# sujeetv/parquet-go

Measured on AMD Instinct MI355X. Metric: decoded GB/s (uncompressed output) per GPU & node at 1/2/4/8; % HBM roofline, higher is better.
Workload: dtype int32; 1 GPU; C2: optional INT32, 100000000 rows x 7 dictionary widths (b=1,2,4,8,12,16,20), ~10% nulls, RLE_DICTIONARY (uniform indices), V1, UNCOMPRESSED, 20000 rows/page; bytes_in=821696760, bytes_out=3220121800, streams=2, parallelism=single GPU

## Files before the change

parquet-go_amd/csrc/pqg_kernels.h:

```cpp
#pragma once
#include <hip/hip_runtime.h>

#include "pqgpu.h"
#include "pqg_common.h"

namespace pqg {

namespace crc { struct Rec; struct TileRec; }
namespace flt { struct Pred; struct Col; struct Sel; }

constexpr int kCrcWaves = 4;
constexpr int kCrcThreads = 64 * kCrcWaves;
constexpr int kBigWaves = 8;
constexpr int kBigDictThreads = 64 * kBigWaves;
constexpr int kExportWaves = 4;
constexpr int kExportThreads = 64 * kExportWaves;
constexpr int kExportGridY = 16;
constexpr int kWalkLanes = kWalkThreads;

__global__ void k_tile_jobs(const JobDev* jobs, int* tile_job);
__global__ void k_page_cands(JobDev* jobs, const int* tile_job, int* tile_count, int* tile_okc, int64_t* cand_pos,
                             int* cand_list, int* cand_total, int region);
__global__ void k_cand_parse(JobDev* jobs, const int* tile_job, const int* cand_list, const int* cand_total, int region,
                             int* tile_okc, const int64_t* cand_pos, Cand* cands);
__global__ void k_tile_scan(JobDev* jobs, const int* tile_count, const int* tile_okc, int* tile_off, int* tile_okoff);
__global__ void k_cand_link(JobDev* jobs, const int* tile_job, int64_t total_tiles, const int* tile_count,
                            const int* tile_off, const int* tile_okoff, const Cand* cands, int* succ, int* idx2slot,
                            int* ok2slot);
__global__ void k_page_chain(JobDev* jobs, PageDev* pages, const Cand* cands, const int* succ, const int* idx2slot,
                             const int* ok2slot, int* order);
__global__ void k_scan_pages(JobDev* jobs, PageDev* pages, int n_jobs, int prewalk, int stride);
__global__ void k_page_list(JobDev* jobs, PageDev* pages, int n_jobs, int* list, int list_cap, int* total,
                            int* queues);
__global__ void k_crc_plan(const JobDev* jobs, const PageDev* pages, const int* list, const int* total, int n_recs,
                           crc::Rec* recs, crc::TileRec* tiles, int tile_cap, int* tile_ctr);
__global__ void k_page_crc(const crc::Rec* recs, const crc::TileRec* tiles, const int* tile_ctr, int tile_cap,
                           int* queue, uint32_t* raws);
__global__ void k_crc_fin(PageDev* pages, const int* list, const int* total, int n_recs, crc::Rec* recs,
                          const uint32_t* raws);
__global__ void k_snap_plan(const JobDev* jobs, PageDev* pages, const int* list, const int* total, int* ctr,
                            SnapSub* subs, int sub_cap, int* seg_page, int seg_cap);
__global__ void k_snap_seg(const JobDev* jobs, const PageDev* pages, const int* seg_page, const int* seg_total,
                           int seg_cap, uint2* F);
__global__ void k_snap_link(const JobDev* jobs, PageDev* pages, const int* list, const int* total, SnapSub* subs,
                            const uint2* F);
__global__ void k_snap_decode(const JobDev* jobs, PageDev* pages, const SnapSub* subs, const int* sub_total,
                              int sub_cap, int* queue, uint8_t* scratch);
__global__ void k_snappy(JobDev* jobs, PageDev* pages, const int* list, const int* total, int* queue,
                         uint8_t* scratch);
__global__ void k_inflate(JobDev* jobs, PageDev* pages, const int* list, const int* total, int* queue,
                          uint8_t* scratch, int mode);
__global__ void k_inflate_s(JobDev* jobs, PageDev* pages, const int* list, const int* total, int* queue,
                            uint8_t* scratch);
__global__ void k_zstd(JobDev* jobs, PageDev* pages, const int* list, const int* total, int* queue, uint8_t* scratch,
                       uint8_t* wspace);
__global__ void k_lz4(JobDev* jobs, PageDev* pages, const int* list, const int* total, int* queue, uint8_t* scratch);
__global__ void k_lz4_batch(JobDev* jobs, PageDev* pages, const int* list, const int* total, int* queue,
                            uint8_t* scratch);
__global__ void k_page_levels(JobDev* jobs, PageDev* pages, const int* list, const int* total, int* queue,
                              uint8_t* scratch, HStream* streams, uint8_t* def_arena, uint8_t* rep_arena,
                              LongLev* longs, int long_cap, LevPiece* pieces, int piece_cap, int split);
__global__ void k_page_levels_w1(JobDev* jobs, PageDev* pages, const int* list, const int* total, int* queue,
                                 uint8_t* scratch, HStream* streams, uint8_t* def_arena, uint8_t* rep_arena,
                                 LongLev* longs, int long_cap, LevPiece* pieces, int piece_cap, int split);
__global__ void k_dict_resolve(JobDev* jobs, int n_jobs, PageDev* pages, uint8_t* scratch);
__global__ void k_level_long(PageDev* pages, const int* ctr, const LongLev* longs, int long_cap,
                             const LevPiece* pieces, int piece_cap, int* queue);
__global__ void k_hybrid_walk(const PageDev* pages, const int* list, const int* total, HStream* streams,
                              RunEnt* runs, BlockDesc* blks, LongWalk* longs, int long_cap);
__global__ void k_walk_long(const int* ctr, const LongWalk* longs, int long_cap, BlockDesc* blks);
__global__ void k_nn_scan_sums(JobDev* jobs, PageDev* pages, uint8_t* scratch, const HStream* streams, NnSums* sums,
                               NnJob* njobs, int* ctr, int64_t parts_cap);
__global__ void k_nn_scan(JobDev* jobs, PageDev* pages, uint8_t* scratch, const HStream* streams, const BlockDesc* blks,
                          int* ctr, PartRec* parts, int64_t parts_cap, const NnSums* sums, const NnJob* njobs);
template <int Mode>
__global__ void k_values(JobDev* jobs, PageDev* pages, const PartRec* parts, const int* total, int* queue,
                         uint8_t* value_arena, const HStream* streams, const RunEnt* runs, const BlockDesc* blks);
__global__ void k_finalize(JobDev* jobs, int n_jobs, const PageDev* pages);
__global__ void k_bss(JobDev* jobs, PageDev* pages, const PartRec* parts, const int* total, int* queue,
                      uint8_t* value_arena);
__global__ void k_dict_idx(JobDev* jobs, PageDev* pages, const PartRec* parts, const int* total, int* queue,
                           uint8_t* value_arena, const HStream* streams, const RunEnt* runs, const BlockDesc* blks);
__global__ void k_dict_export(JobDev* jobs, const PageDev* pages, int64_t* aoffs_arena, uint8_t* dchars_arena);
__global__ void k_dict_plan(JobDev* jobs, PageDev* pages, const PartRec* parts, const int* total,
                            uint8_t* value_arena, const HStream* streams, const RunEnt* runs, const BlockDesc* blks,
                            VRec* recs);
__global__ void k_dict4(PageDev* pages, const int* total, int* queue, const VRec* recs, int big);
__global__ void k_dict4_big(PageDev* pages, const int* total, int* queue, const VRec* recs);
__global__ void k_str_dict(JobDev* jobs, PageDev* pages, int64_t* doffs_arena);
__global__ void k_str_count(JobDev* jobs, PageDev* pages, PartRec* parts, const int* total, int* queue,
                            int64_t* offs_arena, const HStream* streams, const RunEnt* runs, const BlockDesc* blks);
__global__ void k_str_plain(JobDev* jobs, PageDev* pages, const int* list, const int* total, int* queue,
                            int64_t* offs_arena);
__global__ void k_char_scan(JobDev* jobs, PageDev* pages, PartRec* parts, int64_t* offs_arena);
__global__ void k_str_delta(JobDev* jobs, PageDev* pages, const int* list, const int* total, int* queue,
                            int64_t* offs_arena);
__global__ void k_str_dba(JobDev* jobs, PageDev* pages, const int* list, const int* total, int* queue,
                          uint8_t* value_arena, int64_t* offs_arena);
__global__ void k_str_copy(JobDev* jobs, PageDev* pages, const PartRec* parts, const int* total, int* queue,
                           uint8_t* value_arena, int64_t* offs_arena);

int assemble_launch(hipStream_t s, const pqg_assemble_args* a, int64_t* seg_scratch, int64_t* tot);
int list_count_launch(hipStream_t s, const pqg_list_args* a, int64_t* seg_scratch, int64_t* tot);
int list_write_launch(hipStream_t s, const pqg_list_args* a, int64_t* seg_scratch);
int nested_count_launch(hipStream_t s, const pqg_nested_args* a, int64_t* seg_scratch, int64_t* tot);
int nested_write_launch(hipStream_t s, const pqg_nested_args* a, int64_t* seg_scratch, const int64_t* tot);
int pack_levels_launch(hipStream_t s, const uint8_t* levels, int64_t n, int bw, uint8_t* packed);
int filter_launch(hipStream_t s, const flt::Pred& p, const flt::Col& c, const pqg_dictionary* dict, uint32_t* ebits,
                  uint8_t* bitmap, int64_t n, int mode, bool lds, int64_t* seg, int64_t* tot);
int select_launch(hipStream_t s, const flt::Sel& a, int64_t* seg, int64_t* tot);

#ifdef PQG_PROFILE
int prof_read_values(unsigned long long* out);
int prof_read_levels(unsigned long long* out);
int prof_read_strings(unsigned long long* out);
int prof_read_snappy(unsigned long long* out);
int prof_read_dict(unsigned long long* out);
int prof_read_inflate(unsigned long long* out);
int prof_read_bss(unsigned long long* out);
#endif

}
```

parquet-go_amd/csrc/pqg_levdec.h:

```cpp
#pragma once
#include "pqg_common.h"
#include "pqg_device.h"
#include "pqg_hybrid.h"

namespace pqg {

__device__ __forceinline__ int reg_stream(const JobDev& job, const PageDev& pg, HStream* streams, int32_t* slot,
                                          int pidx, int kind, gcu8 p, int64_t n, int w, int64_t count) {
  const int64_t rb = pg.run_off, bb = pg.blk_off;
  const int id = pidx * 3 + (kind > 2 ? 2 : kind);
  HStream& S = streams[id];
  S.p = (const uint8_t*)p;
  S.n = n;
  S.run_base = job.run_base + rb;
  S.blk_base = job.blk_base + bb;
  S.page = pidx;
  S.kind = kind;
  S.w = w;
  S.count = (int32_t)count;
  S.n_runs = 0;
  S.produced = 0;
  S.status = kOK;
  S.n_blocks = 0;
  *slot = id;
// ... 513 lines not shown
        const uint32_t ok = pay < n ? (n - pay + (uint32_t)w - 1) / (uint32_t)w : 0u;
        take = ok * 8;
        status = kEOF;
      }
    }
    if (status != kOK) return status;
    if (take > (uint32_t)kLongLev && longs && defer_long(bp, take, pay, produced)) {
      deferred = true;
      produced += take;
      pos = nx;
      return kOK;
    }
    uint32_t done = 0;
    while (done < take) {
      const uint32_t pre = (uint32_t)(((uintptr_t)out + produced) & 15);
      uint32_t piece = take - done;
      if (piece > (uint32_t)kLSpan - pre) piece = (uint32_t)kLSpan - pre;
      uint32_t info = pay;
      if (bp) {
        const uint64_t b0 = (uint64_t)pay * 8 + (uint64_t)done * (uint32_t)w;
        const uint32_t byte0 = (uint32_t)(b0 >> 3);
        const uint32_t nbytes = (uint32_t)(((uint64_t)piece * (uint32_t)w + 7) >> 3) + 8;
        if (!in_win(byte0, nbytes)) fill(byte0);
        info = 0x80000000u | (uint32_t)(((uint64_t)(byte0 - wbase) << 3) + (b0 & 7));
      }
      if (kW1 || w == 1) {
        bits_clear();
        if ((uint32_t)lane <= (pre + piece - 1) >> 5) bits_or(pre, piece, bp, bp ? (info & 0x7fffffffu) : pay, lane);
        bits_store(produced, piece);
        produced += piece;
        done += piece;
        continue;
      }
      if constexpr (!kW1) {
      PQG_L uint8_t* TM = lds_ptr(sh->tmap);
      *(PQG_L u32x4_t*)(TM + 16 * lane) = u32x4_t{0u, 0u, 0u, 0u};
      __builtin_amdgcn_wave_barrier();
      if (lane == 0) {
        lds_ptr(sh->tent)[0] = u32x2_t{pre, info};
        TM[pre] = 1;
      }
      __builtin_amdgcn_wave_barrier();
      expand(produced, piece);
      produced += piece;
      done += piece;
      }
    }
    pos = nx;
    return kOK;
  }
};

struct LongTables {
  LongLev* longs;
  LevPiece* pieces;
  int* ctr;
  int long_cap, piece_cap;
};

using LevelDecoder = LevelDecoderT<false>;

template <bool kW1 = false>
__device__ __forceinline__ int level_stream(gcu8 p, int64_t n, int w, uint32_t count, gu8 out, uint32_t maxl,
                                            LevShared& sh, uint32_t* nn, const LongTables& lt, int pidx,
                                            bool* deferred = nullptr) {
  LevelDecoderT<kW1> dec{p, (uint32_t)n, kW1 ? 1 : w, count, out, maxl, &sh, lt.longs, lt.pieces, lt.ctr, lt.long_cap,
                         lt.piece_cap, pidx};
  const int e = dec.run();
#ifdef PQG_PROFILE
  for (int k = 0; k < 8; k++) PQG_ACC(k, 0, dec.pacc[k]);
#endif
  *nn = (uint32_t)wave_sum((int64_t)dec.nn);
  if (deferred) *deferred = dec.deferred;
  return e;
}

struct PageStreams {
  gcu8 rep, def;
  int64_t rep_n, def_n;
  int e;
  gcu8 val;
  int64_t val_n;
  int vmode;
};
__device__ __forceinline__ PageStreams page_setup(const JobDev& job, const PageDev& pg, int pidx, PageDev* pages,
                                                  HStream* streams, const int* total, const uint8_t* scratch,
                                                  bool writer) {
  PageStreams r{nullptr, nullptr, -1, -1, kOK, nullptr, 0, -1};
  gcu8 block;
  int64_t blen;
  int32_t levels = 0;
  if (pg.page_type == 3) {
    levels = (int32_t)((uint32_t)pg.rep_len + (uint32_t)pg.def_len);
    blen = (int32_t)((uint32_t)pg.csize - (uint32_t)levels);
    if (pg.scratch_offset >= 0) blen = (int32_t)((uint32_t)pg.usize - (uint32_t)levels);
  } else {
    blen = pg.scratch_offset >= 0 ? pg.usize : pg.csize;
  }
  if (pg.scratch_offset >= 0) block = gconst(scratch) + job.scratch_base + pg.scratch_offset;
  else block = gconst(job.data) + pg.payload_offset + (levels > 0 ? levels : 0);
  int64_t vpos = 0;
  if (pg.page_type == 0) {
    if (job.max_rep > 0) {
      if (blen - vpos < 4) r.e = kEOF;
      else {
        const int64_t sz = rd_u32(block + vpos);
        const int64_t take = min(sz, blen - vpos - 4);
        r.rep = block + vpos + 4;
        r.rep_n = take;
        vpos += 4 + take;
      }
    }
    if (r.e == kOK && job.max_def > 0) {
      if (blen - vpos < 4) r.e = kEOF;
      else {
        const int64_t sz = rd_u32(block + vpos);
        const int64_t take = min(sz, blen - vpos - 4);
        r.def = block + vpos + 4;
        r.def_n = take;
        vpos += 4 + take;
      }
    }
  } else {
    gcu8 lv = gconst(job.data) + pg.payload_offset;
    if (levels > 0 && pg.rep_len > 0) { r.rep = lv; r.rep_n = pg.rep_len; }
    if (levels > 0 && pg.def_len > 0) { r.def = lv + pg.rep_len; r.def_n = levels - pg.rep_len; }
  }
  if (r.e != kOK) {
    if (writer) pages[pidx].read_status = r.e;
    return r;
  }
  if (job.keep_dict && pg.encoding != 8) {
    r.e = kNOT_DICT;
    if (writer) pages[pidx].read_status = r.e;
    return r;
  }
  const int64_t n = pg.num_values;
  const int64_t vn = blen - vpos;
  gcu8 val = block + vpos;
  r.val = val;
  r.val_n = vn;
  r.vmode = job.keep_dict                                              ? kModeIdx
            : pg.encoding == 9 && job.value_width > 0                  ? kModeBss
            : job.value_width == 0 || (pg.encoding == 7 && job.type == 7) ? 2
            : (pg.encoding == 8 && job.value_width == 4)                ? 1
            : pg.encoding == 5                                          ? 3
                                                                        : 0;
  if (writer) {
    PageDev& P = pages[pidx];
    P.block = (const uint8_t*)block;
    P.block_len = blen;
    P.val = (const uint8_t*)val;
    P.val_n = vn;
    P.rep = (const uint8_t*)r.rep;
    P.rep_n = r.rep_n;
    P.def = (const uint8_t*)r.def;
    P.def_n = r.def_n;
    if (pg.encoding == 8 && vn >= 1) {
      const int wv = val[0];
      P.dict_width = wv;
      if (wv >= 1 && wv <= 32 && n > 0) reg_stream(job, pg, streams, &P.hs_val, pidx, 2, val + 1, vn - 1, wv, n);
    } else if (pg.encoding == 3 && job.type == 0 && vn >= 4) {
      const int64_t sz = rd_u32(val);
      const int64_t take = min(sz, vn - 4);
      if (n > 0) reg_stream(job, pg, streams, &P.hs_val, pidx, 3, val + 4, take, 1, n);
    }
    const int vm = r.vmode;
    P.vmode = vm;
    int* present = const_cast<int*>(total) + kModePresentOff;
    if (present[vm] == 0) present[vm] = 1;
    if (vm == 2 && (pg.encoding == 6 || pg.encoding == 7) && present[kPresentDeltaStr] == 0) present[kPresentDeltaStr] = 1;
  }
  return r;
}

}
```

parquet-go_amd/csrc/pqg_levels.hip:

```cpp
#include <hip/hip_runtime.h>

#include "pqg_common.h"
#include "pqg_kernels.h"
#include "pqg_device.h"
#include "pqg_hybrid.h"
#include "pqg_levdec.h"
#include "pqg_lev1.h"
#include <type_traits>

namespace pqg {

#ifndef PQG_LEVELS_WPE
#define PQG_LEVELS_WPE 6
#endif

#ifdef PQG_PROFILE
int prof_read_levels(unsigned long long* out) {
  unsigned long long z[64] = {0};
  if (hipMemcpyFromSymbol(out, HIP_SYMBOL(pqg_prof), sizeof(z)) != hipSuccess) return -1;
  hipMemcpyToSymbol(HIP_SYMBOL(pqg_prof), z, sizeof(z));
  return 0;
}
#endif


#ifndef PQG_LANE_WIN
#define PQG_LANE_WIN 8
#endif
constexpr int kLaneWinG = PQG_LANE_WIN;
struct LaneWin {
  gcu8 p;
  uint32_t n;
  uint32_t base;
  PQG_L uint32_t* r;
  __device__ __forceinline__ void fill(uint32_t pos) {
    const uint32_t mis = (uint32_t)((uintptr_t)(p + pos) & 15);
    base = pos - mis;
    const uintptr_t a0 = (uintptr_t)(p + pos) - mis;
    const uintptr_t last = ((uintptr_t)(p + n) - 1) & ~(uintptr_t)15;
    uint4 g[kLaneWinG];
#pragma unroll
    for (int k = 0; k < kLaneWinG; k++) {
      const uintptr_t a = a0 + 16 * k;
      g[k] = ldg16(a <= last ? a : last);
    }
#pragma unroll
    for (int k = 0; k < kLaneWinG; k++) {
      const uint4 v = mask_tail(g[k], (int64_t)pos - mis + 16 * k, n);
      r[64 * (4 * k + 0)] = v.x;
      r[64 * (4 * k + 1)] = v.y;
      r[64 * (4 * k + 2)] = v.z;
      r[64 * (4 * k + 3)] = v.w;
    }
  }
  __device__ __forceinline__ void ensure(uint32_t pos) {
    if (pos - base > 16 * kLaneWinG - 16) fill(pos);
  }
  __device__ __forceinline__ void read12(uint32_t pos, uint32_t& a, uint32_t& b, uint32_t& c) const {
    const uint32_t off = pos - base;
    const uint32_t d = off >> 2, sh = (off & 3) * 8;
    const uint32_t x0 = r[64 * d], x1 = r[64 * (d + 1)], x2 = r[64 * (d + 2)], x3 = r[64 * (d + 3)];
    a = __builtin_amdgcn_alignbit(x1, x0, sh);
    b = __builtin_amdgcn_alignbit(x2, x1, sh);
    c = __builtin_amdgcn_alignbit(x3, x2, sh);
  }
  __device__ __forceinline__ void peek12(uint32_t pos, uint32_t& a, uint32_t& b, uint32_t& c) {
    ensure(pos);
    read12(pos, a, b, c);
  }
};

__device__ __forceinline__ void sync_ensure(LaneWin& w, bool reads, uint32_t rp) {
  const bool need = reads && rp - w.base > 16 * kLaneWinG - 16;
  if (__ballot(need) != 0 && reads) w.fill(rp);
}

__global__ void __launch_bounds__(kWalkThreads) k_hybrid_walk(const PageDev* pages, const int* list, const int* total,
                                                              HStream* streams, RunEnt* runs, BlockDesc* blks,
                                                              LongWalk* longs, int long_cap) {
  static_assert(kWalkThreads == 64, "LaneWin: dword k of lane L at buf[64 k + L]");
  __shared__ uint32_t buf[4 * kLaneWinG * kWalkThreads];
  const int nt = *total;
  int* const n_long = const_cast<int*>(total) + kCtrLongWalk;
  for (int g = blockIdx.x * kWalkThreads + threadIdx.x; g < nt; g += gridDim.x * kWalkThreads) {
    const PageDev& pg = pages[list[g]];
    const int hs = pg.hs_val;
    if (hs < 0) continue;
    HStream& S = streams[hs];
    const uint32_t w = (uint32_t)S.w;
    const uint32_t n = (uint32_t)S.n, count = (uint32_t)S.count;
    const uint32_t rb = (w + 7) >> 3;
    const uint64_t vmask = rb >= 4 ? 0xffffffffull : ((1ull << (8 * rb)) - 1);
    PQG_G uint32_t* R = (PQG_G uint32_t*)(gmut(runs) + S.run_base);
    PQG_G uint32_t* B = (PQG_G uint32_t*)(gmut(blks) + S.blk_base);
    LaneWin rd{gconst(S.p), n, 0xfffffff0u, lds_ptr(buf) + threadIdx.x};
    if (n > 0) rd.fill(0);
    uint32_t pos = 0, produced = 0, nr = 0;
    int status = kOK;
    uint32_t nb = 0, bv0 = 0, br0 = 0, bn = 0;
    uint64_t blo = ~0ull, bhi = 0;
    auto close_block = [&]() {
      if (bn == 0) return;
      const uint32_t lo = blo == ~0ull ? 0u : (uint32_t)blo;
      const uint32_t nbytes = blo == ~0ull ? 0u : (uint32_t)(bhi - blo);
      PQG_G uint32_t* d = B + 4 * nb;
      stg16((uintptr_t)d, make_uint4(bv0, br0, lo, (nbytes & 0xffff) | (bn << 16)));
      nb++;
    };
    while (produced < count) {
      if (pos >= n) { status = kEOF; break; }
      sync_ensure(rd, true, pos);
      uint32_t xa, xb, xc;
      rd.read12(pos, xa, xb, xc);
      uint64_t x = (uint64_t)xa | (uint64_t)xb << 32;
      uint32_t h, hl;
      if ((x & 0x80) == 0) {
        h = (uint32_t)x & 0x7f;
        hl = 1;
      } else {
        uint64_t v = 0;
        unsigned sft = 0;
        int e = kOK;
        hl = 0;
        for (uint32_t i = 0;; i++) {
          if (pos + i >= n) { e = kEOF; break; }
          uint32_t b;
          if (i < 8) {
            b = (uint32_t)(x >> (8 * i)) & 0xff;
          } else {
            uint32_t ya, yb, yc;
            rd.peek12(pos + i, ya, yb, yc);
            b = ya & 0xff;
          }
          if (b < 0x80) {
            if (i > 9 || (i == 9 && b > 1)) e = kRLE;
            else {
              v |= sft < 64 ? (uint64_t)b << sft : 0;
              if (v > 0x7fffffffull) e = kRLE;
            }
            hl = i + 1;
            break;
          }
          if (sft < 64) v |= (uint64_t)(b & 0x7f) << sft;
          sft += 7;
        }
        if (e) { status = e; break; }
        h = (uint32_t)v;
        {
          uint32_t ya, yb, yc;
          rd.peek12(pos + hl, ya, yb, yc);
          x = ((uint64_t)ya | (uint64_t)yb << 32) << 8;
        }
      }
      pos += hl;
      uint32_t take, st, src;
      const uint32_t left = count - produced;
      if (h & 1) {
        const uint32_t groups = h >> 1;
        if (groups == 0) { status = kRLE; break; }
        take = groups >= (left + 7) >> 3 ? left : groups * 8;
        const uint32_t need = (take + 7) >> 3;
        if ((uint64_t)pos + (uint64_t)(need - 1) * w >= n) {
          const uint32_t ok = pos < n ? (n - pos + w - 1) / w : 0;
          take = ok * 8;
          status = kEOF;
        }
        st = produced | kRunBP;
        src = pos;
        pos = (uint64_t)pos + (uint64_t)groups * w > 0xffffffffull ? 0xffffffffu : pos + groups * w;
      } else {
        const uint32_t cnt = h >> 1;
        if (cnt == 0) { status = kRLE; break; }
        if (pos >= n || n - pos < rb) { status = kEOF; break; }
        src = (uint32_t)((x >> 8) & vmask);
        pos += rb;
        if (w < 32 && (src >> w) != 0) { status = kRLE; break; }
        take = cnt < left ? cnt : left;
        st = produced;
      }
      if (take > 0) {
        stg8((uintptr_t)(R + 2 * nr), st, src);
        const uint32_t rend = produced + take;
        if ((st & kRunBP) && take > (uint32_t)kLongWalk) {
          const uint32_t K = min((uint32_t)kHBlock, ((8u * kHBlockBytes - 14u) / w) & ~7u);
          const uint32_t R = (take + K - 1) / K;
          const int li = atomicAdd(n_long, 1);
          if (li < long_cap) {
            close_block();
            LongWalk L;
            L.blk = S.blk_base + nb;
            L.v0 = produced;
            L.take = take;
            L.run = nr;
            L.src = src;
            L.w = (int32_t)w;
            L.K = (int32_t)K;
            longs[li] = L;
            nb += R;
            bv0 = rend;
            br0 = nr + 1;
            bn = 0;
            blo = ~0ull;
            bhi = 0;
            produced = rend;
            nr++;
            if (status) break;
            continue;
          }
        }
        for (uint32_t v = produced; v < rend;) {
          if (bn == kHBlockRuns || v >= bv0 + kHBlock) {
            close_block();
            bv0 = v;
            br0 = nr;
            bn = 0;
            blo = ~0ull;
            bhi = 0;
          }
          uint32_t pe = rend < bv0 + kHBlock ? rend : bv0 + kHBlock;
          if (st & kRunBP) {
            const uint64_t rbit = (uint64_t)src * 8;
            const uint64_t b0 = (rbit + (uint64_t)(v - produced) * w) >> 3;
            const uint64_t org = blo < b0 ? blo : b0;
            const uint64_t lim = (org + kHBlockBytes) * 8;
            const uint64_t fit = lim > rbit ? (lim - rbit) / w : 0;
            if (produced + fit <= v) {
              close_block();
              bv0 = v;
              br0 = nr;
              bn = 0;
              blo = ~0ull;
              bhi = 0;
              continue;
            }
            if (produced + fit < pe) pe = (uint32_t)(produced + fit);
            const uint64_t b1 = (rbit + (uint64_t)(pe - produced) * w + 7) >> 3;
            blo = org;
            bhi = b1 > bhi ? b1 : bhi;
          }
          bn++;
          v = pe;
        }
        produced = rend;
        nr++;
      }
      if (status) break;
    }
    close_block();
    S.n_runs = (int32_t)nr;
    S.produced = (int32_t)produced;
    S.status = status;
    S.n_blocks = (int32_t)nb;
  }
}

__global__ void __launch_bounds__(256) k_walk_long(const int* ctr, const LongWalk* longs, int long_cap,
                                                   BlockDesc* blks) {
  const int n = min(ctr[kCtrLongWalk], long_cap);
  const uint32_t tid = blockIdx.x * 256 + threadIdx.x, stride = gridDim.x * 256;
  for (int r = 0; r < n; r++) {
    const LongWalk L = longs[r];
    const uint32_t R = (L.take + (uint32_t)L.K - 1) / (uint32_t)L.K;
    for (uint32_t j = tid; j < R; j += stride) {
      const uint32_t a = j * (uint32_t)L.K;
      const uint32_t cnt = min((uint32_t)L.K, L.take - a);
      const uint64_t bit0 = (uint64_t)L.src * 8 + (uint64_t)a * (uint32_t)L.w;
      const uint64_t lo = bit0 >> 3, hi = (bit0 + (uint64_t)cnt * (uint32_t)L.w + 7) >> 3;
      stg16((uintptr_t)(blks + L.blk + j),
            make_uint4(L.v0 + a, L.run, (uint32_t)lo, (uint32_t)(hi - lo) | (1u << 16)));
    }
  }
}

__global__ void __launch_bounds__(64) k_level_long(PageDev* pages, const int* ctr, const LongLev* longs, int long_cap,
                                                   const LevPiece* pieces, int piece_cap, int* queue) {
  const int lane = lane_id();
  const int np = min(ctr[kCtrLevPieces], piece_cap);
  for (;;) {
    const int t = queue_next(queue);
    if (t >= np) return;
    const LevPiece pc = pieces[t];
    if (pc.run < 0 || pc.run >= long_cap) continue;
    const LongLev L = longs[pc.run];
    if (pages[L.pidx].decode_status != kOK) continue;
    const uintptr_t ob = (uintptr_t)L.out;
    const uint32_t mask = (1u << L.w) - 1;
    const int64_t navail = L.p ? (int64_t)(L.end - L.p) : 0;
    uint32_t nn = 0;
    const uintptr_t a0 = (ob + pc.v0) & ~(uintptr_t)15;
    for (uintptr_t a = a0 + 16 * (uintptr_t)lane; a < ob + pc.v1; a += 1024) {
      const int64_t i0 = (int64_t)(a - ob);
      uint32_t v[16];
      if (L.p) {
        const int64_t ib = i0 < 0 ? 0 : i0;
        const int64_t bit = ib * L.w;
        const gcu8 p = gconst(L.p);
        const uint64_t x0 = load_u64_masked(p, navail, bit >> 3, navail);
        const uint64_t x1 = load_u64_masked(p, navail, (bit >> 3) + 8, navail);
        const uint32_t sh = (uint32_t)(bit & 7);
        const int64_t shift0 = (i0 < 0 ? -i0 : 0) * L.w;
#pragma unroll
        for (int k = 0; k < 16; k++) {
          const int64_t b = (int64_t)sh + (int64_t)k * L.w - shift0;
          uint32_t x = 0;
          if (b >= 0) {
            x = b < 64 ? (uint32_t)(x0 >> b) | (b > 56 ? (uint32_t)(x1 << (64 - b)) : 0u) : (uint32_t)(x1 >> (b - 64));
          }
          v[k] = x & mask;
        }
      } else {
#pragma unroll
        for (int k = 0; k < 16; k++) v[k] = L.value;
      }
      uint32_t wv[4];
#pragma unroll
      for (int k = 0; k < 4; k++) wv[k] = v[4 * k] | v[4 * k + 1] << 8 | v[4 * k + 2] << 16 | v[4 * k + 3] << 24;
      if (i0 >= (int64_t)pc.v0 && i0 + 16 <= (int64_t)pc.v1) {
        stg16o(a, make_uint4(wv[0], wv[1], wv[2], wv[3]));
#pragma unroll
        for (int k = 0; k < 16; k++) nn += v[k] == (uint32_t)L.maxl;
      } else {
#pragma unroll
        for (int k = 0; k < 16; k++) {
          if (i0 + k >= (int64_t)pc.v0 && i0 + k < (int64_t)pc.v1) {
            *(PQG_G uint8_t*)(a + k) = (uint8_t)v[k];
            nn += v[k] == (uint32_t)L.maxl;
          }
        }
      }
    }
    const int64_t tot = wave_sum((int64_t)nn);
    if (lane == 0 && L.maxl <= 255 && tot) atomicAdd(&pages[L.pidx].not_null, (int32_t)tot);
  }
}

__device__ __forceinline__ bool w1_job(const JobDev& job) { return job.max_rep == 0 && job.max_def <= 1; }

union LevW1Shared {
  LevShared lev;
  Lev1Shared l1;
};
template <bool kW1>
using LevelsShared = typename std::conditional<kW1, LevW1Shared, LevShared>::type;
__device__ __forceinline__ LevShared& lev_sh(LevShared& s) { return s; }
__device__ __forceinline__ LevShared& lev_sh(LevW1Shared& s) { return s.lev; }

template <bool kW1>
__device__ __forceinline__ void page_levels(JobDev* jobs, PageDev* pages, const int* list, const int* total, int* queue,
                                            uint8_t* scratch, HStream* streams, uint8_t* def_arena, uint8_t* rep_arena,
                                            LongLev* longs, int long_cap, LevPiece* pieces, int piece_cap, int split_flags) {
  __shared__ __attribute__((aligned(16))) LevelsShared<kW1> shu;
  LevShared& sh = lev_sh(shu);
  const int split = split_flags & 1;
  const bool whole = kW1 && (split_flags & 2);
  const int lane = lane_id();
  const LongTables lt{longs, pieces, const_cast<int*>(total), long_cap, piece_cap};
  for (;;) {
    const int t = queue_next(queue);
    if (t >= *total) return;
    const int pidx = __builtin_amdgcn_readfirstlane(list[t]);
    const PageDev pg = pages[pidx];
    const JobDev job = jobs[pg.job];
    if (split && w1_job(job) != kW1) continue;
    if (lane == 0) {
      pages[pidx].hs_rep = pages[pidx].hs_def = pages[pidx].hs_val = -1;
      pages[pidx].vmode = -1;
    }
    if (pg.read_status != kOK || (pg.page_type != 0 && pg.page_type != 3)) continue;
    if (job.status == kCAPACITY) continue;
    const PageStreams ps = page_setup(job, pg, pidx, pages, streams, total, scratch, lane == 0);
    if (ps.e != kOK) continue;
    const int64_t n = pg.num_values;
    int64_t nn = 0;
    int de = kOK;
    if (n > 0) {
      if (!kW1 && job.max_rep > 0) {
        if (ps.rep_n < 0) de = kLEVELS;
        else {
          uint32_t unused;
          de = level_stream<kW1>(ps.rep, ps.rep_n, bits_len((uint32_t)job.max_rep), (uint32_t)n,
                                 gmut(rep_arena) + job.slot_base + pg.slot_offset, 0x100u, sh, &unused, lt, pidx);
        }
      }
      if (de == kOK) {
        if (job.max_def > 0) {
          if (ps.def_n < 0) de = kLEVELS;
          else {
            uint32_t c = 0;
            bool done = false;
            if constexpr (kW1) {
              if (whole && job.max_def == 1 && ps.def_n <= kL1MaxN)
                done = lev1_page(ps.def, (uint32_t)ps.def_n, (uint32_t)n,
                                 gmut(def_arena) + job.slot_base + pg.slot_offset, shu.l1, &c);
            }
            if (done) de = kOK;
            else
              de = level_stream<kW1>(ps.def, ps.def_n, bits_len((uint32_t)job.max_def), (uint32_t)n,
                                     gmut(def_arena) + job.slot_base + pg.slot_offset, (uint32_t)job.max_def, sh, &c,
                                     lt, pidx);
            nn = c;
          }
        } else {
          nn = n;
        }
      }
    }
    if (lane == 0) {
      pages[pidx].not_null = de == kOK ? (int32_t)nn : 0;
      if (de != kOK) pages[pidx].decode_status = de;
    }
  }
}

__global__ void __launch_bounds__(64, PQG_LEVELS_WPE) k_page_levels(JobDev* jobs, PageDev* pages, const int* list, const int* total,
                                                    int* queue, uint8_t* scratch, HStream* streams,
                                                    uint8_t* def_arena, uint8_t* rep_arena, LongLev* longs,
                                                    int long_cap, LevPiece* pieces, int piece_cap, int split) {
  page_levels<false>(jobs, pages, list, total, queue, scratch, streams, def_arena, rep_arena, longs, long_cap, pieces,
                     piece_cap, split);
}

#ifndef PQG_LEVELS_W1_WPE
#define PQG_LEVELS_W1_WPE 4
#endif
__global__ void __launch_bounds__(64, PQG_LEVELS_W1_WPE) k_page_levels_w1(JobDev* jobs, PageDev* pages, const int* list,
                                                       const int* total, int* queue, uint8_t* scratch,
                                                       HStream* streams, uint8_t* def_arena, uint8_t* rep_arena,
                                                       LongLev* longs, int long_cap, LevPiece* pieces, int piece_cap,
                                                       int split) {
  page_levels<true>(jobs, pages, list, total, queue, scratch, streams, def_arena, rep_arena, longs, long_cap, pieces,
                    piece_cap, split);
}

__device__ void plan_parts(JobDev& job, int np, bool fail, const PageDev* pp, const HStream* streams,
                           const BlockDesc* blks, int* ctr, PartRec* parts, int64_t cap, int64_t* part);

__device__ void resolve_dictionary(JobDev& job, PageDev* pages, uint8_t* scratch) {
  int np = job.num_pages < job.page_cap ? job.num_pages : job.page_cap;
  if (job.status == kCAPACITY) np = 0;
  if (job.dict_page < 0 || job.dict_page >= np) return;
  PageDev& dp = pages[job.page_base + job.dict_page];
  if (dp.read_status != kOK) return;
  const uint8_t* blk =
      dp.scratch_offset >= 0 ? scratch + job.scratch_base + dp.scratch_offset : job.data + dp.payload_offset;
  const int64_t blen = dp.usize;
  const int64_t cnt = dp.num_values;
  const int w = job.keep_dict ? job.entry_width : job.value_width;
  dp.block = blk;
  dp.block_len = blen;
  int st = kOK;
  int flags = 0;
  if (w > 0) {
    if (job.type == 3) {
      const int64_t full = blen / 12, rem = blen % 12;
      if (cnt > full + (rem > 0 ? 1 : 0)) st = kEOF;
      else if (cnt == full + 1 && rem > 0) flags = 1;
    } else if (cnt * w > blen) {
      st = kEOF;
    }
  } else {
    flags = 2;
    job.need_doffs = (cnt < blen / 4 ? cnt : blen / 4) + 2;
    if (job.need_doffs > job.doffs_cap) job.status = kCAPACITY;
    if (job.keep_dict) {
      job.need_dchars = blen;
      if (blen > job.dchars_cap) job.status = kCAPACITY;
    }
  }
  if (st == kOK) {
    job.flags |= flags;
    job.dict_data = blk;
    job.dict_count = (flags & 2) ? 0 : cnt;
    job.dict_len = blen;
  } else {
    dp.read_status = st;
  }
}

__global__ void __launch_bounds__(256) k_dict_resolve(JobDev* jobs, int n_jobs, PageDev* pages, uint8_t* scratch) {
  const int j = blockIdx.x * 256 + threadIdx.x;
  if (j < n_jobs) resolve_dictionary(jobs[j], pages, scratch);
}

__device__ int nn_job_tail(JobDev& job, PageDev* pages, uint8_t* scratch, int np, int64_t carry, bool fail0) {
  int cap = fail0 || job.status == kCAPACITY;
  job.num_values = carry;
  const int64_t vb = job.value_width > 0 ? carry * job.value_width : 0;
  if (job.value_width > 0 && vb > job.value_cap) job.status = kCAPACITY, cap = 1;
  job.values_bytes = vb;
  return cap;
}

__device__ int64_t part_n(const PageDev& pg, const HStream* streams, int64_t* count, bool* hyb);
__device__ void plan_split_pages(JobDev& job, const PageDev* pp, const HStream* streams, const BlockDesc* blks,
                                 PartRec* parts, int64_t base, int nbig, const int* big, const int64_t* boff);
__device__ void plan_parts_from(JobDev& job, int np, const PageDev* pp, const HStream* streams, const BlockDesc* blks,
                                PartRec* parts, int64_t base);

__device__ __forceinline__ int nn_pages(const JobDev& job) {
  const int np = job.num_pages < job.page_cap ? job.num_pages : job.page_cap;
  return job.status == kCAPACITY ? 0 : np;
}

__device__ __forceinline__ void nn_page_counts(const PageDev* pp, int i, int np, const HStream* streams, int32_t* nn,
                                               int32_t* kv, int32_t* vmode) {
  const PageDev& pg = pp[i < np ? i : np - 1];
  const int32_t f_type = pg.page_type, f_nn = pg.not_null, f_rs = pg.read_status, f_ds = pg.decode_status,
                f_enc = pg.encoding, vm = pg.vmode;
  *nn = *kv = 0;
  *vmode = vm;
  if (i >= np) return;
  const bool data = f_type == 0 || f_type == 3;
  *nn = data ? f_nn : 0;
  int32_t k = 0;
// ... 293 lines not shown
```

parquet-go_amd/csrc/pqg_runtime.hip:

```cpp
#include <hip/hip_runtime.h>
#include <cstdlib>

#include <algorithm>
#include <cstring>
#include <type_traits>
#include <vector>

#include "pqg_ctx.h"
#include "pqg_crc.h"
#include "pqg_kernels.h"
#include "pqg_zstd.h"

using namespace pqg;

namespace {

constexpr int kMaxAttempts = 6;

JobKey job_key(const pqg_chunk_job& j) {
  return JobKey{(uintptr_t)j.data, j.total_compressed_size, j.num_values_hint, (j.col.flags & PQG_COL_KEEP_DICT) ? 1 : 0};
}

int64_t align_up(int64_t v, int64_t a) { return (v + a - 1) / a * a; }

// ... 301 lines not shown
  PageDev* pages = (PageDev*)c->pages.p;
  int* list = (int*)c->list.p;
  int* ctr = (int*)c->counters.p;
  auto Q = [&](int k) { return ctr + kQueueBase + k * kQueueInts; };
  uint8_t* scratch = (uint8_t*)c->scratch.p;
  const int waves = c->num_cus * 20;
  hipStream_t s = c->stream;
  if (c->timed) hipEventRecord(c->ev[0], s);
  hipMemsetAsync(ctr + kQueueBase, 0, sizeof(int) * kQueueSlots * kQueueInts, s);
  const int64_t nt = c->total_tiles;
  int* tcount = (int*)c->tile_count.p;
  int* toff = (int*)c->tile_off.p;
  Cand* cands = (Cand*)c->cands.p;
  int* tokc = (int*)c->tile_okc.p;
  int* tokoff = (int*)c->tile_okoff.p;
  if (b.prewalk) hipLaunchKernelGGL(k_scan_pages, dim3(n), dim3(64), 0, s, jobs, pages, n, kPrewalkPages, (int)c->stride);
  if (nt > 0) {
    int64_t* cpos = (int64_t*)c->cand_pos.p;
    int* clist = (int*)c->cand_list.p;
    const int region = (int)((nt + kQShards - 1) / kQShards) * kCandPerTile;
    hipLaunchKernelGGL(k_tile_jobs, dim3(n, (unsigned)std::min(c->tile_blocks, 64)), dim3(256), 0, s, jobs, (int*)c->tile_job.p);
    hipLaunchKernelGGL(k_page_cands, dim3((unsigned)nt), dim3(256), 0, s, jobs, (const int*)c->tile_job.p, tcount, tokc,
                       cpos, clist, Q(kQueueCands),
                       region);
    hipLaunchKernelGGL(k_cand_parse, dim3((unsigned)std::min<int64_t>((nt * kCandPerTile + 255) / 256, c->num_cus * 4)),
                       dim3(256), 0, s, jobs, (const int*)c->tile_job.p, clist, Q(kQueueCands), region, tokc, cpos, cands);
  }
  const dim3 tile_grid(n, (unsigned)c->tile_blocks), page_grid(n, (unsigned)c->page_blocks);
  hipLaunchKernelGGL(k_tile_scan, tile_grid, dim3(1024), 0, s, jobs, tcount, tokc, toff, tokoff);
  if (nt > 0)
    hipLaunchKernelGGL(k_cand_link, dim3((unsigned)((nt * kCandPerTile + 255) / 256)), dim3(256), 0, s, jobs,
                       (const int*)c->tile_job.p, nt,
                       tcount, toff, tokoff, cands, (int*)c->succ.p, (int*)c->idx2slot.p, (int*)c->ok2slot.p);
  hipLaunchKernelGGL(k_page_chain, page_grid, dim3(1024), 0, s, jobs, pages, cands, (const int*)c->succ.p,
                     (const int*)c->idx2slot.p, (const int*)c->ok2slot.p, (int*)c->order.p);
  hipLaunchKernelGGL(k_scan_pages, dim3(n), dim3(64), 0, s, jobs, pages, n, 0, 0);
  if (c->timed) hipEventRecord(c->ev[1], s);
  hipLaunchKernelGGL(k_page_list, page_grid, dim3(1024), 0, s, jobs, pages, n, list,
                     (int)std::min<int64_t>(c->list_cap, INT32_MAX), ctr, ctr + kCtrZeroed);
  if (c->timed) hipEventRecord(c->ev[2], s);
  c->crc_ran = c->verify_crc;
  c->crc_timed = c->verify_crc && c->timed;
  if (c->verify_crc) {
    crc::Rec* recs = (crc::Rec*)c->crc_recs.p;
    crc::TileRec* ctiles = (crc::TileRec*)c->crc_tiles.p;
    uint32_t* raws = (uint32_t*)c->crc_raws.p;
    int* tile_ctr = Q(kQueueCrc) + kCrcTileCtr;
    const unsigned page_waves = (unsigned)std::max<int64_t>(1, std::min<int64_t>(c->list_cap, (int64_t)c->num_cus * 16));
    if (c->timed) hipEventRecord(c->ev_crc[0], s);
    hipLaunchKernelGGL(k_crc_plan, dim3(page_waves), dim3(64), 0, s, jobs, pages, list, ctr, 0, recs, ctiles,
                       (int)c->crc_tile_cap, tile_ctr);
    hipLaunchKernelGGL(k_page_crc, dim3(qgrid((int64_t)c->num_cus * c->crc_per_cu)), dim3(kCrcThreads), 0, s, recs, ctiles, tile_ctr,
                       (int)c->crc_tile_cap, Q(kQueueCrc), raws);
    hipLaunchKernelGGL(k_crc_fin, dim3(page_waves), dim3(64), 0, s, pages, list, ctr, 0, recs, raws);
    if (c->timed) hipEventRecord(c->ev_crc[1], s);
  }
  if (b.any_snappy) {
    const SnapTables T{(SnapSub*)c->sn_subs.p, (int)std::min<int64_t>(c->sn_sub_cap, INT32_MAX), (int*)c->sn_segpage.p,
                       (int)std::min<int64_t>(c->sn_seg_cap, INT32_MAX), (uint2*)c->sn_F.p};
    launch_snappy(c, s, jobs, pages, list, ctr, c->list_cap, ctr + kCtrSnapSplit, Q(kQueueSnapSplit), Q(kQueueSnapSerial),
                  scratch, T);
  }
  if (b.any_gzip) {
    hipLaunchKernelGGL(k_inflate_s, dim3(qgrid(c->num_cus * c->inflate_per_cu)), dim3(64), 0, s, jobs, pages, list, ctr,
                       Q(kQueueInflate), scratch);
    hipLaunchKernelGGL(k_inflate, dim3(qgrid(c->num_cus * 4)), dim3(64), 0, s, jobs, pages, list, ctr,
                       Q(kQueueInflateRedo), scratch, 1);
  }
  if (b.any_zstd)
    hipLaunchKernelGGL(k_zstd, dim3(zstd_grid(c)), dim3(64), 0, s, jobs, pages, list, ctr, Q(kQueueZstd), scratch,
                       (uint8_t*)c->zstd_ws.p);
  if (b.any_lz4)
    hipLaunchKernelGGL(c->lz4_batch ? k_lz4_batch : k_lz4, dim3(qgrid((int64_t)c->num_cus * c->lz4_per_cu)), dim3(64), 0, s, jobs, pages, list, ctr,
                       Q(kQueueLz4), scratch);
  if (c->timed) hipEventRecord(c->ev[3], s);
  HStream* streams = (HStream*)c->streams.p;
  RunEnt* runs = (RunEnt*)c->runs.p;
  BlockDesc* blks = (BlockDesc*)c->blks.p;
  LongLev* llong = (LongLev*)c->lev_long.p;
  LevPiece* lpieces = (LevPiece*)c->lev_pieces.p;
  const int llc = (int)std::min<int64_t>(c->lev_long_cap, INT32_MAX), lpc = (int)std::min<int64_t>(c->lev_piece_cap, INT32_MAX);
  hipLaunchKernelGGL(k_dict_resolve, dim3((unsigned)((n + 255) / 256)), dim3(256), 0, s, jobs, n, pages, scratch);
  const int split = b.any_w1 && b.any_gen;
  if (b.any_w1)
    hipLaunchKernelGGL(k_page_levels_w1, dim3(qgrid(c->num_cus * 32)), dim3(64), 0, s, jobs, pages, list, ctr,
                       Q(kQueueLevels), scratch, streams, (uint8_t*)c->def_arena.p, (uint8_t*)c->rep_arena.p, llong, llc,
                       lpieces, lpc, split | (c->lev1 ? 2 : 0));
  if (b.any_gen)
    hipLaunchKernelGGL(k_page_levels, dim3(qgrid(c->num_cus * 24)), dim3(64), 0, s, jobs, pages, list, ctr,
                       Q(split ? kQueueLevGen : kQueueLevels), scratch, streams, (uint8_t*)c->def_arena.p,
                       (uint8_t*)c->rep_arena.p, llong, llc, lpieces, lpc, split);
  if (b.any_levels)
    hipLaunchKernelGGL(k_level_long, dim3(qgrid(c->num_cus * c->levlong_waves)), dim3(64), 0, s, pages, ctr, llong, llc, lpieces, lpc,
                       Q(kQueueLevLong));
  if (c->timed) hipEventRecord(c->ev[4], s);
  const unsigned walk_blocks = (unsigned)std::max<int64_t>(
      1, std::min<int64_t>((c->list_cap + kWalkLanes - 1) / kWalkLanes, c->num_cus * (2048 / kWalkLanes)));
  LongWalk* wlong = (LongWalk*)c->walk_long.p;
  const int wlc = (int)std::min<int64_t>(c->walk_long_cap, INT32_MAX);
  hipLaunchKernelGGL(k_hybrid_walk, dim3(walk_blocks), dim3(kWalkLanes), 0, s, pages, list, ctr, streams, runs, blks,
                     wlong, wlc);
  hipLaunchKernelGGL(k_walk_long, dim3(c->num_cus * 2), dim3(256), 0, s, ctr, wlong, wlc, blks);
  if (c->timed) hipEventRecord(c->ev[5], s);
  if (c->timed) hipEventRecord(c->ev[6], s);
  PartRec* parts = (PartRec*)c->parts.p;
  NnSums* nsums = (NnSums*)c->nn_sums.p;
  NnJob* njobs = (NnJob*)c->nn_jobs.p;
  hipLaunchKernelGGL(k_nn_scan_sums, page_grid, dim3(1024), 0, s, jobs, pages, scratch, streams, nsums, njobs, ctr,
                     c->parts_cap);
  hipLaunchKernelGGL(k_nn_scan, page_grid, dim3(1024), 0, s, jobs, pages, scratch, streams, blks, ctr, parts, c->parts_cap,
                     nsums, njobs);
  if (c->timed) hipEventRecord(c->ev[7], s);
  const int64_t items_cap = c->parts_cap;
  if (!b.any_w4) {
  } else if (c->dict4) {
    VRec* recs = (VRec*)c->vrecs.p;
    hipLaunchKernelGGL(k_dict_plan, dim3((unsigned)std::max<int64_t>(1, std::min<int64_t>((items_cap + 255) / 256, c->num_cus * 4))),
                       dim3(256), 0, s, jobs, pages, parts, ctr, (uint8_t*)c->value_arena.p, streams, runs, blks, recs);
    hipLaunchKernelGGL(k_dict4, dim3(qgrid(c->num_cus * c->dict4_per_cu)), dim3(c->dict4_threads), 0, s, pages, ctr,
                       Q(kQueueDict4), recs, (int)c->dict_big);
    if (c->dict_big)
      hipLaunchKernelGGL(k_dict4_big, dim3(qgrid(c->num_cus)), dim3(kBigDictThreads), 0, s, pages, ctr,
                         Q(kQueueDictBig), recs);
  } else
    hipLaunchKernelGGL(k_values<1>, dim3(qgrid(waves)), dim3(64), 0, s, jobs, pages, parts, ctr, Q(kQueueDict4),
                       (uint8_t*)c->value_arena.p, streams, runs, blks);
  if (b.any_fixed_other) {
    hipLaunchKernelGGL(k_values<0>, dim3(qgrid(waves)), dim3(64), 0, s, jobs, pages, parts, ctr, Q(kQueueValues),
                       (uint8_t*)c->value_arena.p, streams, runs, blks);
    hipLaunchKernelGGL(k_values<3>, dim3(qgrid(waves)), dim3(64), 0, s, jobs, pages, parts, ctr, Q(kQueueDbp),
                       (uint8_t*)c->value_arena.p, streams, runs, blks);
    hipLaunchKernelGGL(k_bss, dim3(qgrid(waves)), dim3(64), 0, s, jobs, pages, parts, ctr, Q(kQueueBss),
                       (uint8_t*)c->value_arena.p);
  }
  auto launch_dict_idx = [&]() {
    hipLaunchKernelGGL(k_dict_idx, dim3(qgrid(waves)), dim3(64), 0, s, jobs, pages, parts, ctr, Q(kQueueDictIdx),
                       (uint8_t*)c->value_arena.p, streams, runs, blks);
  };
  if (b.any_keep && !b.any_keep_var) launch_dict_idx();
  if (c->timed) hipEventRecord(c->ev[8], s);
  if (b.any_var)
    hipLaunchKernelGGL(k_str_dict, dim3(n), dim3(512), 0, s, jobs, pages, (int64_t*)c->doffs_arena.p);
  if (b.any_keep_var) {
    launch_dict_idx();
    hipLaunchKernelGGL(k_dict_export, dim3(n, kExportGridY), dim3(kExportThreads), 0, s, jobs, pages,
                       (int64_t*)c->aoffs_arena.p, (uint8_t*)c->dchars_arena.p);
  }
  if (b.any_var_out) {
    int64_t* offs = (int64_t*)c->offs_arena.p;
    hipLaunchKernelGGL(k_str_plain, dim3(qgrid(c->num_cus * 4 * 512 / kPwThreads)), dim3(kPwThreads), 0, s, jobs, pages, list, ctr,
                       Q(kQueueStrPlain), offs);
    hipLaunchKernelGGL(k_str_count, dim3(qgrid(waves)), dim3(64), 0, s, jobs, pages, parts, ctr, Q(kQueueStrCount), offs,
                       streams, runs, blks);
    hipLaunchKernelGGL(k_str_delta, dim3(qgrid(c->num_cus * 8)), dim3(64), 0, s, jobs, pages, list, ctr,
                       Q(kQueueStrDelta), offs);
    hipLaunchKernelGGL(k_char_scan, dim3(n), dim3(256), 0, s, jobs, pages, parts, offs);
    hipLaunchKernelGGL(k_str_copy, dim3(qgrid(c->num_cus * 4)), dim3(512), 0, s, jobs, pages, parts, ctr,
                       Q(kQueueStrCopy), (uint8_t*)c->value_arena.p, offs);
    hipLaunchKernelGGL(k_str_dba, dim3(qgrid(c->num_cus * 6)), dim3(64), 0, s, jobs, pages, list, ctr,
                       Q(kQueueStrDba), (uint8_t*)c->value_arena.p, offs);
  }
  if (c->timed) hipEventRecord(c->ev[9], s);
  hipLaunchKernelGGL(k_finalize, page_grid, dim3(1024), 0, s, jobs, n, pages);
  if (c->timed) hipEventRecord(c->ev[10], s);
  return hip_ok(hipGetLastError());
}

static BatchTraits batch_traits(const pqg_ctx* c, const pqg_chunk_job* jobs, int n_jobs) {
  BatchTraits b;
  for (int i = 0; i < n_jobs; i++) {
    const pqg_column_desc& d = jobs[i].col;
    const int width = value_width_of(d);
    b.prewalk |= c->many_pages.find(job_key(jobs[i])) == c->many_pages.end();
    b.any_snappy |= d.codec == PQG_CODEC_SNAPPY;
    b.any_gzip |= d.codec == PQG_CODEC_GZIP;
    b.any_zstd |= d.codec == PQG_CODEC_ZSTD;
    b.any_lz4 |= d.codec == PQG_CODEC_LZ4_RAW;
    (d.max_rep == 0 && d.max_def <= 1 ? b.any_w1 : b.any_gen) = true;
    b.any_levels |= d.max_def > 0 || d.max_rep > 0;
    if (d.flags & PQG_COL_KEEP_DICT) {
      b.any_keep = true;
      b.any_keep_var |= width == 0;
      b.any_var |= width == 0;
      continue;
// ... 269 lines not shown
```

Measured before the change: 1479 GB/s.

## Fuse hybrid-walk of dictionary index streams into the w1 page-levels kernel

Moves the hybrid RLE/bit-packed walk into the width-1 levels kernel: workers first take walk work items (64 pages per item) from the shared queue, doing page setup and the stream walk themselves, then go on to level decoding. The walk no longer reads HStream fields set by the levels pass. It uses values returned by page_setup, so the walk and level decoding no longer have to run in order. This drops one kernel launch and the serialization between the two stages, letting walk and level work overlap within a single queue. In exchange, page_setup runs twice per page, the LDS union grows to hold the walk buffer, and register pressure may rise in the fused kernel.

```diff
diff --git a/parquet-go_amd/csrc/pqg_kernels.h b/parquet-go_amd/csrc/pqg_kernels.h
--- a/parquet-go_amd/csrc/pqg_kernels.h
+++ b/parquet-go_amd/csrc/pqg_kernels.h
@@ -62,12 +62,14 @@
                               LongLev* longs, int long_cap, LevPiece* pieces, int piece_cap, int split);
 __global__ void k_page_levels_w1(JobDev* jobs, PageDev* pages, const int* list, const int* total, int* queue,
                                  uint8_t* scratch, HStream* streams, uint8_t* def_arena, uint8_t* rep_arena,
-                                 LongLev* longs, int long_cap, LevPiece* pieces, int piece_cap, int split);
+                                 LongLev* longs, int long_cap, LevPiece* pieces, int piece_cap, int split,
+                                 RunEnt* runs, BlockDesc* blks, LongWalk* wlongs, int wlong_cap);
 __global__ void k_dict_resolve(JobDev* jobs, int n_jobs, PageDev* pages, uint8_t* scratch);
 __global__ void k_level_long(PageDev* pages, const int* ctr, const LongLev* longs, int long_cap,
                              const LevPiece* pieces, int piece_cap, int* queue);
-__global__ void k_hybrid_walk(const PageDev* pages, const int* list, const int* total, HStream* streams,
-                              RunEnt* runs, BlockDesc* blks, LongWalk* longs, int long_cap);
+__global__ void k_hybrid_walk(const JobDev* jobs, PageDev* pages, const int* list, const int* total,
+                              const uint8_t* scratch, HStream* streams, RunEnt* runs, BlockDesc* blks, LongWalk* longs,
+                              int long_cap);
 __global__ void k_walk_long(const int* ctr, const LongWalk* longs, int long_cap, BlockDesc* blks);
 __global__ void k_nn_scan_sums(JobDev* jobs, PageDev* pages, uint8_t* scratch, const HStream* streams, NnSums* sums,
                                NnJob* njobs, int* ctr, int64_t parts_cap);
diff --git a/parquet-go_amd/csrc/pqg_levdec.h b/parquet-go_amd/csrc/pqg_levdec.h
--- a/parquet-go_amd/csrc/pqg_levdec.h
+++ b/parquet-go_amd/csrc/pqg_levdec.h
@@ -619,11 +619,33 @@
   gcu8 val;
   int64_t val_n;
   int vmode;
+  int hs_val, hs_w;
+  gcu8 hs_p;
+  int64_t hs_n;
 };
+
+__device__ __forceinline__ PageDev page_scan_fields(const PageDev& g) {
+  PageDev pg{};
+  pg.payload_offset = g.payload_offset;
+  pg.slot_offset = g.slot_offset;
+  pg.scratch_offset = g.scratch_offset;
+  pg.page_type = g.page_type;
+  pg.encoding = g.encoding;
+  pg.num_values = g.num_values;
+  pg.csize = g.csize;
+  pg.usize = g.usize;
+  pg.def_len = g.def_len;
+  pg.rep_len = g.rep_len;
+  pg.job = g.job;
+  pg.read_status = g.read_status;
+  pg.run_off = g.run_off;
+  pg.blk_off = g.blk_off;
+  return pg;
+}
 __device__ __forceinline__ PageStreams page_setup(const JobDev& job, const PageDev& pg, int pidx, PageDev* pages,
                                                   HStream* streams, const int* total, const uint8_t* scratch,
                                                   bool writer) {
-  PageStreams r{nullptr, nullptr, -1, -1, kOK, nullptr, 0, -1};
+  PageStreams r{nullptr, nullptr, -1, -1, kOK, nullptr, 0, -1, -1, 0, nullptr, 0};
   gcu8 block;
   int64_t blen;
   int32_t levels = 0;
@@ -696,11 +718,17 @@
     if (pg.encoding == 8 && vn >= 1) {
       const int wv = val[0];
       P.dict_width = wv;
-      if (wv >= 1 && wv <= 32 && n > 0) reg_stream(job, pg, streams, &P.hs_val, pidx, 2, val + 1, vn - 1, wv, n);
+      if (wv >= 1 && wv <= 32 && n > 0) {
+        r.hs_val = reg_stream(job, pg, streams, &P.hs_val, pidx, 2, val + 1, vn - 1, wv, n);
+        r.hs_p = val + 1, r.hs_n = vn - 1, r.hs_w = wv;
+      }
     } else if (pg.encoding == 3 && job.type == 0 && vn >= 4) {
       const int64_t sz = rd_u32(val);
       const int64_t take = min(sz, vn - 4);
-      if (n > 0) reg_stream(job, pg, streams, &P.hs_val, pidx, 3, val + 4, take, 1, n);
+      if (n > 0) {
+        r.hs_val = reg_stream(job, pg, streams, &P.hs_val, pidx, 3, val + 4, take, 1, n);
+        r.hs_p = val + 4, r.hs_n = take, r.hs_w = 1;
+      }
     }
     const int vm = r.vmode;
     P.vmode = vm;
diff --git a/parquet-go_amd/csrc/pqg_levels.hip b/parquet-go_amd/csrc/pqg_levels.hip
--- a/parquet-go_amd/csrc/pqg_levels.hip
+++ b/parquet-go_amd/csrc/pqg_levels.hip
@@ -28,6 +28,8 @@
 #define PQG_LANE_WIN 8
 #endif
 constexpr int kLaneWinG = PQG_LANE_WIN;
+static_assert(kWalkThreads == 64, "LaneWin: dword k of lane L at buf[64 k + L]");
+constexpr int kWalkBufDwords = 4 * kLaneWinG * kWalkThreads;
 struct LaneWin {
   gcu8 p;
   uint32_t n;
@@ -75,25 +77,30 @@
   if (__ballot(need) != 0 && reads) w.fill(rp);
 }
 
-__global__ void __launch_bounds__(kWalkThreads) k_hybrid_walk(const PageDev* pages, const int* list, const int* total,
-                                                              HStream* streams, RunEnt* runs, BlockDesc* blks,
-                                                              LongWalk* longs, int long_cap) {
-  static_assert(kWalkThreads == 64, "LaneWin: dword k of lane L at buf[64 k + L]");
-  __shared__ uint32_t buf[4 * kLaneWinG * kWalkThreads];
-  const int nt = *total;
+__device__ __forceinline__ void walk_item(int g, int nt, const JobDev* jobs, PageDev* pages, const int* list,
+                                          const int* total, const uint8_t* scratch, HStream* streams, RunEnt* runs,
+                                          BlockDesc* blks, LongWalk* longs, int long_cap, uint32_t* buf) {
   int* const n_long = const_cast<int*>(total) + kCtrLongWalk;
-  for (int g = blockIdx.x * kWalkThreads + threadIdx.x; g < nt; g += gridDim.x * kWalkThreads) {
-    const PageDev& pg = pages[list[g]];
-    const int hs = pg.hs_val;
-    if (hs < 0) continue;
+  if (g < nt) {
+    const int pidx = list[g];
+    const PageDev pg = page_scan_fields(pages[pidx]);
+    const JobDev& job = jobs[pg.job];
+    pages[pidx].hs_rep = pages[pidx].hs_def = pages[pidx].hs_val = -1;
+    pages[pidx].vmode = -1;
+    if (pg.read_status != kOK || (pg.page_type != 0 && pg.page_type != 3)) return;
+    if (job.status == kCAPACITY) return;
+    const PageStreams ps = page_setup(job, pg, pidx, pages, streams, total, scratch, true);
+    const int hs = ps.hs_val;
+    if (ps.e != kOK || hs < 0) return;
     HStream& S = streams[hs];
-    const uint32_t w = (uint32_t)S.w;
-    const uint32_t n = (uint32_t)S.n, count = (uint32_t)S.count;
+    const uint32_t w = (uint32_t)ps.hs_w;
+    const uint32_t n = (uint32_t)ps.hs_n, count = (uint32_t)pg.num_values;
+    const int64_t blk_base = job.blk_base + pg.blk_off;
     const uint32_t rb = (w + 7) >> 3;
     const uint64_t vmask = rb >= 4 ? 0xffffffffull : ((1ull << (8 * rb)) - 1);
-    PQG_G uint32_t* R = (PQG_G uint32_t*)(gmut(runs) + S.run_base);
-    PQG_G uint32_t* B = (PQG_G uint32_t*)(gmut(blks) + S.blk_base);
-    LaneWin rd{gconst(S.p), n, 0xfffffff0u, lds_ptr(buf) + threadIdx.x};
+    PQG_G uint32_t* R = (PQG_G uint32_t*)(gmut(runs) + job.run_base + pg.run_off);
+    PQG_G uint32_t* B = (PQG_G uint32_t*)(gmut(blks) + blk_base);
+    LaneWin rd{ps.hs_p, n, 0xfffffff0u, lds_ptr(buf) + lane_id()};
     if (n > 0) rd.fill(0);
     uint32_t pos = 0, produced = 0, nr = 0;
     int status = kOK;
@@ -188,7 +195,7 @@
           if (li < long_cap) {
             close_block();
             LongWalk L;
-            L.blk = S.blk_base + nb;
+            L.blk = blk_base + nb;
             L.v0 = produced;
             L.take = take;
             L.run = nr;
@@ -252,6 +259,16 @@
     S.status = status;
     S.n_blocks = (int32_t)nb;
   }
+}
+
+__global__ void __launch_bounds__(kWalkThreads) k_hybrid_walk(const JobDev* jobs, PageDev* pages, const int* list,
+                                                              const int* total, const uint8_t* scratch,
+                                                              HStream* streams, RunEnt* runs, BlockDesc* blks,
+                                                              LongWalk* longs, int long_cap) {
+  __shared__ uint32_t buf[kWalkBufDwords];
+  const int nt = *total;
+  for (int g0 = blockIdx.x * kWalkThreads; g0 < nt; g0 += gridDim.x * kWalkThreads)
+    walk_item(g0 + (int)threadIdx.x, nt, jobs, pages, list, total, scratch, streams, runs, blks, longs, long_cap, buf);
 }
 
 __global__ void __launch_bounds__(256) k_walk_long(const int* ctr, const LongWalk* longs, int long_cap,
@@ -339,6 +356,13 @@
 union LevW1Shared {
   LevShared lev;
   Lev1Shared l1;
+  uint32_t walk[kWalkBufDwords];
+};
+struct WalkTables {
+  RunEnt* runs;
+  BlockDesc* blks;
+  LongWalk* longs;
+  int long_cap;
 };
 template <bool kW1>
 using LevelsShared = typename std::conditional<kW1, LevW1Shared, LevShared>::type;
@@ -348,27 +372,31 @@
 template <bool kW1>
 __device__ __forceinline__ void page_levels(JobDev* jobs, PageDev* pages, const int* list, const int* total, int* queue,
                                             uint8_t* scratch, HStream* streams, uint8_t* def_arena, uint8_t* rep_arena,
-                                            LongLev* longs, int long_cap, LevPiece* pieces, int piece_cap, int split_flags) {
+                                            LongLev* longs, int long_cap, LevPiece* pieces, int piece_cap, int split_flags,
+                                            const WalkTables& wt) {
   __shared__ __attribute__((aligned(16))) LevelsShared<kW1> shu;
   LevShared& sh = lev_sh(shu);
   const int split = split_flags & 1;
   const bool whole = kW1 && (split_flags & 2);
   const int lane = lane_id();
   const LongTables lt{longs, pieces, const_cast<int*>(total), long_cap, piece_cap};
-  for (;;) {
-    const int t = queue_next(queue);
-    if (t >= *total) return;
-    const int pidx = __builtin_amdgcn_readfirstlane(list[t]);
-    const PageDev pg = pages[pidx];
+  const int nt = *total;
+  const int nwalk = kW1 ? (nt + kWalkThreads - 1) / kWalkThreads : 0;
+  int t = queue_next(queue);
+  if constexpr (kW1) {
+    for (; t < nwalk; t = queue_next(queue))
+      walk_item(t * kWalkThreads + lane, nt, jobs, pages, list, total, scratch, streams, wt.runs, wt.blks, wt.longs,
+                wt.long_cap, shu.walk);
+  }
+  for (;; t = queue_next(queue)) {
+    if (t >= nwalk + nt) return;
+    const int pidx = __builtin_amdgcn_readfirstlane(list[t - nwalk]);
+    const PageDev pg = page_scan_fields(pages[pidx]);
     const JobDev job = jobs[pg.job];
     if (split && w1_job(job) != kW1) continue;
-    if (lane == 0) {
-      pages[pidx].hs_rep = pages[pidx].hs_def = pages[pidx].hs_val = -1;
-      pages[pidx].vmode = -1;
-    }
     if (pg.read_status != kOK || (pg.page_type != 0 && pg.page_type != 3)) continue;
     if (job.status == kCAPACITY) continue;
-    const PageStreams ps = page_setup(job, pg, pidx, pages, streams, total, scratch, lane == 0);
+    const PageStreams ps = page_setup(job, pg, pidx, pages, streams, total, scratch, false);
     if (ps.e != kOK) continue;
     const int64_t n = pg.num_values;
     int64_t nn = 0;
@@ -417,7 +445,7 @@
                                                     uint8_t* def_arena, uint8_t* rep_arena, LongLev* longs,
                                                     int long_cap, LevPiece* pieces, int piece_cap, int split) {
   page_levels<false>(jobs, pages, list, total, queue, scratch, streams, def_arena, rep_arena, longs, long_cap, pieces,
-                     piece_cap, split);
+                     piece_cap, split, WalkTables{nullptr, nullptr, nullptr, 0});
 }
 
 #ifndef PQG_LEVELS_W1_WPE
@@ -427,9 +455,10 @@
                                                        const int* total, int* queue, uint8_t* scratch,
                                                        HStream* streams, uint8_t* def_arena, uint8_t* rep_arena,
                                                        LongLev* longs, int long_cap, LevPiece* pieces, int piece_cap,
-                                                       int split) {
+                                                       int split, RunEnt* runs, BlockDesc* blks, LongWalk* wlongs,
+                                                       int wlong_cap) {
   page_levels<true>(jobs, pages, list, total, queue, scratch, streams, def_arena, rep_arena, longs, long_cap, pieces,
-                    piece_cap, split);
+                    piece_cap, split, WalkTables{runs, blks, wlongs, wlong_cap});
 }
 
 __device__ void plan_parts(JobDev& job, int np, bool fail, const PageDev* pp, const HStream* streams,
diff --git a/parquet-go_amd/csrc/pqg_runtime.hip b/parquet-go_amd/csrc/pqg_runtime.hip
--- a/parquet-go_amd/csrc/pqg_runtime.hip
+++ b/parquet-go_amd/csrc/pqg_runtime.hip
@@ -407,10 +407,18 @@
   const int llc = (int)std::min<int64_t>(c->lev_long_cap, INT32_MAX), lpc = (int)std::min<int64_t>(c->lev_piece_cap, INT32_MAX);
   hipLaunchKernelGGL(k_dict_resolve, dim3((unsigned)((n + 255) / 256)), dim3(256), 0, s, jobs, n, pages, scratch);
   const int split = b.any_w1 && b.any_gen;
-  if (b.any_w1)
+  LongWalk* wlong = (LongWalk*)c->walk_long.p;
+  const int wlc = (int)std::min<int64_t>(c->walk_long_cap, INT32_MAX);
+  if (b.any_w1) {
     hipLaunchKernelGGL(k_page_levels_w1, dim3(qgrid(c->num_cus * 32)), dim3(64), 0, s, jobs, pages, list, ctr,
                        Q(kQueueLevels), scratch, streams, (uint8_t*)c->def_arena.p, (uint8_t*)c->rep_arena.p, llong, llc,
-                       lpieces, lpc, split | (c->lev1 ? 2 : 0));
+                       lpieces, lpc, split | (c->lev1 ? 2 : 0), runs, blks, wlong, wlc);
+  } else {
+    const unsigned walk_blocks = (unsigned)std::max<int64_t>(
+        1, std::min<int64_t>((c->list_cap + kWalkLanes - 1) / kWalkLanes, c->num_cus * (2048 / kWalkLanes)));
+    hipLaunchKernelGGL(k_hybrid_walk, dim3(walk_blocks), dim3(kWalkLanes), 0, s, jobs, pages, list, ctr, scratch, streams,
+                       runs, blks, wlong, wlc);
+  }
   if (b.any_gen)
     hipLaunchKernelGGL(k_page_levels, dim3(qgrid(c->num_cus * 24)), dim3(64), 0, s, jobs, pages, list, ctr,
                        Q(split ? kQueueLevGen : kQueueLevels), scratch, streams, (uint8_t*)c->def_arena.p,
@@ -419,12 +427,6 @@
     hipLaunchKernelGGL(k_level_long, dim3(qgrid(c->num_cus * c->levlong_waves)), dim3(64), 0, s, pages, ctr, llong, llc, lpieces, lpc,
                        Q(kQueueLevLong));
   if (c->timed) hipEventRecord(c->ev[4], s);
-  const unsigned walk_blocks = (unsigned)std::max<int64_t>(
-      1, std::min<int64_t>((c->list_cap + kWalkLanes - 1) / kWalkLanes, c->num_cus * (2048 / kWalkLanes)));
-  LongWalk* wlong = (LongWalk*)c->walk_long.p;
-  const int wlc = (int)std::min<int64_t>(c->walk_long_cap, INT32_MAX);
-  hipLaunchKernelGGL(k_hybrid_walk, dim3(walk_blocks), dim3(kWalkLanes), 0, s, pages, list, ctr, streams, runs, blks,
-                     wlong, wlc);
   hipLaunchKernelGGL(k_walk_long, dim3(c->num_cus * 2), dim3(256), 0, s, ctr, wlong, wlc, blks);
   if (c->timed) hipEventRecord(c->ev[5], s);
   if (c->timed) hipEventRecord(c->ev[6], s);
```

Result: faster. 1496 GB/s (median of 6 runs) (+1.2%).
